# benjamincjackson/distance

Hardware: AMD Instinct MI355X
Metric: pairwise comparisons/sec (higher is better)
Workload: dtype u32

## Files before the change

distance_amd/_lib.py:

```python
from __future__ import annotations

import ctypes as C
import os
import re

_HERE = os.path.dirname(os.path.abspath(__file__))
LIB_PATH = os.environ.get("DST_LIB_PATH") or os.path.join(_HERE, "libdistance_hip.so")
HEADER_PATH = os.path.join(os.path.dirname(_HERE), "include", "distance_hip.h")

_u8p = C.POINTER(C.c_uint8)
_u32p = C.POINTER(C.c_uint32)
_u64p = C.POINTER(C.c_uint64)
_vp = C.c_void_p
ALLGATHER_FN = C.CFUNCTYPE(C.c_int, C.c_void_p, C.c_void_p, C.c_void_p, C.c_size_t, C.c_void_p)
SLAB_SINK = C.CFUNCTYPE(C.c_int, C.c_void_p, C.c_uint64, C.c_uint64, C.c_uint64, C.c_uint64, C.c_void_p)


class LaunchInfo(C.Structure):
    _fields_ = [("path", C.c_int), ("measure", C.c_int), ("family", C.c_int), ("out_kind", C.c_int), ("wide", C.c_int),
                ("square", C.c_int), ("event_waves", C.c_int), ("heavy_events", C.c_int), ("rows_per_tile", C.c_uint32),
                ("tile_cols", C.c_uint32), ("tiles", C.c_uint64), ("hot", C.c_int), ("run_records", C.c_int),
                ("variant", C.c_int), ("ksplit", C.c_uint32), ("pairs", C.c_uint64), ("events_per_pair", C.c_double),
                ("list_length", C.c_double), ("run_adds", C.c_double)]

# ... 54 lines not shown
    "dst_stream_open": (C.c_int, [_vp, C.c_int, C.c_int, C.c_size_t, C.c_int, C.POINTER(_vp)]),
    "dst_stream_open_wire": (C.c_int, [_vp, C.c_int, C.c_int, C.c_size_t, C.c_int, C.c_int, C.POINTER(_vp)]),
    "dst_stream_acquire": (C.c_int, [_vp, C.POINTER(_vp), C.POINTER(C.c_size_t), C.POINTER(_vp)]),
    "dst_stream_submit": (C.c_int, [_vp, C.c_size_t, C.c_int]),
    "dst_stream_collect": (C.c_int, [_vp, C.POINTER(C.c_size_t), C.POINTER(_vp)]),
    "dst_stream_in_flight": (C.c_int, [_vp]),
    "dst_stream_close": (C.c_int, [_vp]),
    "dst_comm_unique_id": (C.c_int, [_vp, C.c_size_t]),
    "dst_comm_create": (C.c_int, [_vp, _vp, C.c_int, C.c_int, C.POINTER(_vp)]),
    "dst_comm_create_custom": (C.c_int, [_vp, C.c_int, C.c_int, ALLGATHER_FN, _vp, C.POINTER(_vp)]),
    "dst_comm_destroy": (C.c_int, [_vp]),
    "dst_upload_shared": (C.c_int, [_vp, C.c_int, _vp, C.c_size_t, C.c_size_t, C.c_size_t, C.c_int, _vp]),
    "dst_shared_range": (C.c_int, [C.c_uint64, C.c_int, C.c_int, _u64p, _u64p]),
    "dst_shared_block_layout": (C.c_int, [C.c_uint64, C.c_int, C.c_uint32, _u32p]),
    "dst_shared_stats": (C.c_int, [_vp, C.c_int, _u64p, _u64p, _u64p]),
    "dst_comm_info": (C.c_int, [_vp, C.POINTER(C.c_int), C.POINTER(C.c_int)]),
    "dst_gather_slabs": (C.c_int, [_vp, _vp, _vp, _u64p, _u64p, C.c_int, _vp]),
    "dst_nearest": (C.c_int, [_vp, C.c_int, C.c_int, C.c_int, C.c_int, C.c_uint32, _vp, _vp, _vp, C.c_size_t, _u32p]),
    "dst_clusters": (C.c_int, [_vp, C.c_int, C.c_double, C.c_uint64, _vp, C.c_size_t, _u64p, _u64p]),
    "dst_nj": (C.c_int, [_vp, C.c_int, C.c_uint64, _vp, _vp, C.c_size_t]),
    "dst_nj_matrix": (C.c_int, [_vp, _vp, C.c_uint64, _vp, _vp, C.c_size_t]),
    "dst_newick": (C.c_int, [C.c_uint64, _vp, _vp, C.c_char_p, _vp, _vp, C.c_size_t, C.POINTER(C.c_size_t)]),
    "dst_newick_support": (C.c_int, [C.c_uint64, _vp, _vp, C.c_char_p, _vp, _vp, _vp, C.c_size_t,
                                     C.POINTER(C.c_size_t)]),
    "dst_bootstrap_columns": (None, [C.c_uint64, C.c_uint32, C.c_uint64, _vp]),
    "dst_nj_bootstrap": (C.c_int, [_vp, C.c_int, _vp, C.c_size_t, C.c_size_t, C.c_size_t, C.c_uint32, C.c_uint64,
                                   C.c_uint64, _vp, _vp, _vp, C.c_size_t]),
    "dst_host_alloc": (C.c_int, [C.c_size_t, C.POINTER(_vp)]),
    "dst_host_free": (C.c_int, [_vp]),
    "dst_out_bytes": (C.c_size_t, [C.c_int, C.c_int, C.c_uint64]),
# ... 35 lines not shown
```

distance_amd/csrc/dst_api.cpp:

```cpp
#include <algorithm>
#include <cmath>
#include <cstdio>
#include <cstdlib>
#include <cstring>
#include <memory>
#include <mutex>
#include <new>
#include <vector>

#include "dst_ctx.h"

using namespace dst;

namespace dst {

std::string g_create_err;
std::mutex g_create_mu;

int publish_prep(dst_ctx *ctx, hipStream_t stream);
int wait_for_other_runs(dst_ctx *ctx, hipStream_t stream);

int fail(dst_ctx *ctx, int status, const std::string &msg)
{
    if (ctx)
        ctx->err = msg;
    return status;
}

int fail_hip(dst_ctx *ctx, hipError_t e, const char *what)
{
    return fail(ctx, e == hipErrorOutOfMemory ? DST_ERR_NOMEM : DST_ERR_HIP,
                std::string(what) + ": " + hipGetErrorString(e));
}

// ... 88 lines not shown
            HIP_TRY(ctx, hipFree(b));
    s.ref.planes = nullptr;
    s.ref.hot_planes = nullptr;
    s.ref.hot_sites = nullptr;
    s.ref.stats = nullptr;
    s.ref.partials = nullptr;
    HIP_TRY(ctx, hipMalloc((void **)&s.ref.planes, 4 * s.nchunks * sizeof(uint4)));
    HIP_TRY(ctx, hipMalloc((void **)&s.ref.hot_planes, s.nchunks * sizeof(uint4)));
    HIP_TRY(ctx, hipMalloc((void **)&s.ref.hot_sites, s.nchunks * kChunkSites * sizeof(uint32_t)));
    HIP_TRY(ctx, hipMalloc((void **)&s.ref.stats, 8 * sizeof(uint64_t)));
    HIP_TRY(ctx, hipMalloc((void **)&s.ref.partials, s.nchunks * 16 * sizeof(uint32_t)));
    s.ref.nchunks = s.nchunks;
    return DST_OK;
}

bool planes_deferred_by_pack()
{
    static const bool keep = std::getenv("DST_PACK_ALL_PLANES") != nullptr;
    return !keep;
}

int pack_queue(dst_ctx *ctx, DeviceSet &s, const uint8_t *d_codes, size_t n, size_t len, size_t row_stride,
               const uint32_t *d_counts, unsigned long long *d_first_bad, hipStream_t stream, bool want_lists, bool nibbles)
{
    if (nibbles)
        want_lists = false;
    int rc = shape_set(ctx, s, n, len);
    if (rc)
        return rc;
    PackLists pl{};
    if (want_lists) {
        rc = alloc_ref(ctx, s);
        if (!rc && s.rec.pre_cap < n + 1) {
            if (s.rec.pre_cold)
                HIP_TRY(ctx, hipFree(s.rec.pre_cold));
            s.rec.pre_cold = s.rec.pre_hot = nullptr;
            s.rec.pre_totals = nullptr;
            s.rec.pre_cap = 0;
            const size_t words = 5 * (n + 1) + 8 + ((2 * (n + 1)) & 1);
            HIP_TRY(ctx, hipMalloc((void **)&s.rec.pre_cold, words * sizeof(uint32_t)));
            s.rec.pre_cap = n + 1;
        }
        if (!rc && s.runs.n_alloc < n + 1) {
            if (s.runs.index)
// ... 27 lines not shown
        pl.cnt_cold = s.rec.pre_cold;
        pl.cnt_hot = s.rec.pre_hot;
        pl.slots = s.rec.pre_slots;
        pl.defer_planes = planes_deferred_by_pack() ? 1 : 0;
        static const bool no_runs = std::getenv("DST_NO_RUN_RECORDS") != nullptr;
        if (!no_runs) {
            pl.cnt_run = s.runs.cnt_run;
            pl.run_cold = s.runs.run_cold;
            pl.run_hot = s.runs.run_hot;
        }
    }
    if (!want_lists)
        HIP_TRY(ctx, hipMemsetAsync(d_first_bad, 0xFF, sizeof(unsigned long long), stream));
    if (int rc_t = timer_begin(ctx, 1, stream))
        return rc_t;
    if (nibbles)
        HIP_TRY(ctx, launch_pack_nibbles(d_codes, row_stride, s, d_first_bad, stream));
    else
        HIP_TRY(ctx, launch_pack(d_codes, row_stride, s, d_first_bad, want_lists ? &pl : nullptr, stream));
    if (int rc_t = timer_end(ctx, 1, stream))
        return rc_t;
    if (d_counts) {
        HIP_TRY(ctx, hipMemsetAsync(s.counts, 0, s.npad * 4 * sizeof(uint32_t), stream));
        HIP_TRY(ctx, hipMemcpyAsync(s.counts, d_counts, n * 4 * sizeof(uint32_t),
                                    hipMemcpyDeviceToDevice, stream));
        s.have_counts = true;
    }
    return DST_OK;
}

int invalid_code_error(dst_ctx *ctx, unsigned long long first_bad, size_t len)
{
    char msg[160];
    std::snprintf(msg, sizeof msg,
// ... 6 lines not shown

int pack_set(dst_ctx *ctx, DeviceSet &s, const uint8_t *d_codes, size_t n, size_t len, size_t row_stride,
             const uint32_t *d_counts, hipStream_t stream);

int pack_from_device(dst_ctx *ctx, int slot, const uint8_t *d_codes, size_t n, size_t len,
                     size_t row_stride, const uint32_t *d_counts, hipStream_t stream)
{
    return pack_set(ctx, ctx->set[slot], d_codes, n, len, row_stride, d_counts, stream);
}

int pack_set(dst_ctx *ctx, DeviceSet &s, const uint8_t *d_codes, size_t n, size_t len, size_t row_stride,
             const uint32_t *d_counts, hipStream_t stream)
{
    const bool want_lists = ctx->path != DST_PATH_DENSE && n >= 2 && len > 0 && n < kEntryMask && len < kSiteMask &&
                            0.5 * (double)n * (double)n * (double)len >= ctx->prep_min_work;
    int rc = pack_queue(ctx, s, d_codes, n, len, row_stride, d_counts, ctx->d_first_bad, stream, want_lists);
    if (rc)
        return rc;
    const uint32_t max_run = (uint32_t)std::min<uint64_t>(n / 3, 24000000000ull / (32ull * std::max<size_t>(n, 1)));
    HIP_TRY(ctx, launch_report(ctx->d_first_bad,
                               want_lists ? reinterpret_cast<const unsigned long long *>(s.ref.stats) : nullptr,
                               want_lists ? s.rec.pre_cold : nullptr, want_lists ? s.rec.pre_hot : nullptr, n, ctx->d_report, stream,
                               want_lists ? &s.runs : nullptr, max_run, want_lists ? s.rec.pre_totals : nullptr));
    HIP_TRY(ctx, hipStreamSynchronize(stream));
    const unsigned long long first_bad = ctx->h_report[0], totals[2] = {ctx->h_report[9], ctx->h_report[10]};
    if (want_lists)
        for (int k = 0; k < 8; ++k)
            s.ref.h_stats[k] = ctx->h_report[1 + k];
    if (first_bad != ~0ull)
        return invalid_code_error(ctx, first_bad, len);
    s.loaded = true;
    if (want_lists) {
        s.ref.valid = true;
        const double max_dev = kListsMaxDeviation * (double)len * (double)std::min<size_t>(n, kRefSamples);
        s.rec.pre_valid = (double)s.ref.h_stats[1] <= (double)(unsigned long long)max_dev;
        s.lean = s.rec.pre_valid;
        s.planes_deferred = s.rec.pre_valid && planes_deferred_by_pack();
        s.rec.pre_epoch = s.epoch;
        s.rec.pre_total_cold = totals[0];
        s.rec.pre_total_hot = totals[1];
        s.runs.n_run = s.rec.pre_valid ? (uint32_t)ctx->h_report[11] : 0u;
        s.runs.removed = s.runs.n_run ? ctx->h_report[12] : 0;
        s.runs.active = s.runs.n_run != 0;
        s.runs.corr_family = -1;
    }
    return DST_OK;
}

int ensure_planes(dst_ctx *ctx, DeviceSet &s, hipStream_t stream)
{
    if (!s.planes_deferred)
        return DST_OK;
    if (s.partial)
        return fail(ctx, DST_ERR_STATE, "a set uploaded with dst_upload_shared runs on the consensus path only (its planes are "
                                        "not stored)");
    int rc = wait_for_other_runs(ctx, stream);
    if (rc)
        return rc;
    HIP_TRY(ctx, launch_planes_from_slots(s, stream));
// ... 873 lines not shown
                    ctx->text_num, (void *)ctx->text_len, (void *)ctx->text_scan, (void *)ctx->text_buf, (void *)ctx->text_flag, ctx->text_ties,
                    (void *)ctx->ids[0].off, (void *)ctx->ids[0].chars, (void *)ctx->ids[1].off, (void *)ctx->ids[1].chars, ctx->nn_slab, ctx->nn_lists,
                    ctx->cl_slab, ctx->cl_work})
        if (b)
            (void)hipFree(b);
    if (ctx->scratch)
        (void)hipFree(ctx->scratch);
    if (ctx->text_ties_host)
        (void)hipHostFree(ctx->text_ties_host);
    if (ctx->scratch_free)
        (void)hipEventDestroy(ctx->scratch_free);
    if (ctx->hot_free)
        (void)hipEventDestroy(ctx->hot_free);
    if (ctx->prep_event)
        (void)hipEventDestroy(ctx->prep_event);
    for (auto &r : ctx->recent)
        if (r.event)
            (void)hipEventDestroy(r.event);
    if (ctx->d_first_bad)
        (void)hipFree(ctx->d_first_bad);
    if (ctx->h_report)
        (void)hipHostFree(ctx->h_report);
    for (auto &t : ctx->timer)
        for (int k = 0; k < dst_ctx::kTimerRing; ++k) {
            if (t.begin[k])
                (void)hipEventDestroy(t.begin[k]);
            if (t.end[k])
                (void)hipEventDestroy(t.end[k]);
        }
    if (ctx->stream)
// ... 62 lines not shown
    plan_consensus_launch(measure, out_kind, wide != 0, square != 0, n_rows_in_launch, n_cols, total_pairs, events_per_pair,
                          list_length, run_adds, hot != 0, info);
    info->path = hot ? DST_PATH_HYBRID : DST_PATH_CONSENSUS;
    return DST_OK;
}

int dst_run_records(const dst_ctx *ctx, int slot, uint64_t *run_records, uint64_t *entries_removed)
{
    if (!ctx || slot < 0 || slot > 1)
        return DST_ERR_ARG;
    const DeviceSet &s = ctx->set[slot];
    if (run_records)
        *run_records = s.runs.active ? s.runs.n_run : 0;
    if (entries_removed)
        *entries_removed = s.runs.active ? s.runs.removed : 0;
    return DST_OK;
}

int dst_planes_stored(const dst_ctx *ctx, int slot, int *stored)
{
    if (!ctx || slot < 0 || slot > 1 || !stored)
        return DST_ERR_ARG;
    *stored = ctx->set[slot].loaded && !ctx->set[slot].planes_deferred ? 1 : 0;
    return DST_OK;
}

int dst_set_variant(dst_ctx *ctx, int variant)
{
    if (!ctx || variant < 0)
        return DST_ERR_ARG;
// ... 932 lines not shown
```

distance_amd/csrc/dst_consensus.hip:

```cpp
#include "dst_device.hpp"

#ifndef DST_OVF_DEPTH
#define DST_OVF_DEPTH 2
#endif

namespace dst {
namespace {

__device__ __forceinline__ int ref_class(uint32_t nib)
{
    return nib == 8 ? 0 : nib == 4 ? 1 : nib == 2 ? 2 : nib == 1 ? 3 : 4;
}

__device__ __forceinline__ uint32_t popc4(uint4 v)
{
    return __builtin_popcount(v.x) + __builtin_popcount(v.y) + __builtin_popcount(v.z) + __builtin_popcount(v.w);
}

__device__ __forceinline__ uint32_t sample_record(uint32_t k, uint32_t n, uint32_t samples)
{
    static_assert(kRefSamples == 512, "shifts below");
    return samples == n ? k : k * (n >> 9) + ((k * (n & 511u)) >> 9);
}

// ... 380 lines not shown
        sum += __shfl_xor(sum, 1);
        sum += __shfl_xor(sum, 2);
        sum += __shfl_xor(sum, 4);
        if (lane == 0 && sum)
            atomicAdd(total, (unsigned long long)sum);
    }
}

template <uint32_t CLN, bool WITHOUT_HOT>
__global__ __launch_bounds__(256) void slot_fill_kernel(const uint4 *__restrict__ slots, const uint4 *__restrict__ planes,
                                                        const uint4 *__restrict__ ref_planes,
                                                        const uint4 *__restrict__ hot_planes, uint32_t n,
                                                        uint32_t nchunks, uint32_t npad,
                                                        const uint32_t *__restrict__ rec_off, uint32_t *__restrict__ rec_ent,
                                                        uint32_t *__restrict__ range_start, uint32_t rec_first, uint32_t ent_cap,
                                                        const uint32_t *__restrict__ run_index, const uint32_t *__restrict__ run_state)
{
    constexpr uint32_t RLN = 64u / CLN;
    const uint32_t lane = threadIdx.x & 63u, wave = blockIdx.x * 4u + (threadIdx.x >> 6);
    const uint32_t rl = lane % RLN, cl = lane / RLN;
    const uint32_t r = rec_first + wave * RLN + rl;
    const bool live = r < n;
    const size_t ps = (size_t)nchunks * npad;
    uint32_t run = 0;
    const uint32_t base0 = live ? rec_off[r - rec_first] : 0u;
    const bool run_record = live && run_state && run_state[1] != 0 && run_index[r] != 0xFFFFFFFFu;
    const uint4 zero4 = make_uint4(0, 0, 0, 0);
    uint4 nslot = (live && cl < nchunks) ? slots[(size_t)cl * npad + r] : zero4;
    uint4 nslot2 = (live && cl + CLN < nchunks) ? slots[(size_t)(cl + CLN) * npad + r] : zero4;
    for (uint32_t c0 = 0; c0 < nchunks; c0 += CLN) {
        const uint32_t c = c0 + cl;
        const uint4 slot = nslot;
// ... 72 lines not shown
                }
            }
        }
        run += tot;
    }
}

constexpr uint32_t kBucketThreads = 1024;

constexpr uint32_t kBucketWalk = 8;
__global__ __launch_bounds__(kBucketThreads) void site_bucket_kernel(const uint32_t *__restrict__ rec_off,
                                                                     const uint32_t *__restrict__ rec_ent,
                                                                     const uint32_t *__restrict__ range_start, uint32_t n,
                                                                     uint32_t npad, uint32_t n_sites, uint4 *__restrict__ site_inl,
                                                                     uint32_t *__restrict__ site_ent,
                                                                     uint32_t *__restrict__ ovf_total)
{
    constexpr uint32_t NT = kBucketThreads, RPT = kPanelCols / NT;
    static_assert(NT == kBucketSites, "one bucket per thread in the offset scan");
    static_assert(RPT * NT == kPanelCols, "every record of the panel has its thread");
    __shared__ uint32_t cnt[kBucketSites];
    __shared__ uint32_t ooff[kBucketSites];
    __shared__ __attribute__((aligned(16))) uint16_t tabl[kBucketSites][16];
    __shared__ uint32_t wave_tot[NT / 64];
    __shared__ uint32_t blk_base;
    __shared__ uint32_t long_n, long_from[kPanelCols], long_to[kPanelCols];
    __shared__ uint16_t long_rec[kPanelCols];
    const uint32_t panel = blockIdx.y, tid = threadIdx.x, lane = tid & 63u;
    const uint32_t s0 = blockIdx.x * kBucketSites, ns = min(kBucketSites, n_sites - s0);
    const uint32_t r0 = panel * kPanelCols, nrec = min(kPanelCols, n - r0);
    cnt[tid] = 0;
    if (tid == 0)
// ... 321 lines not shown
        if ((threadIdx.x & 63u) == 0)
            part[threadIdx.x >> 6][k] = v[k];
    }
    __syncthreads();
    if (threadIdx.x < 4) {
        const unsigned long long t = part[0][threadIdx.x] + part[1][threadIdx.x] + part[2][threadIdx.x] + part[3][threadIdx.x];
        if (t)
            atomicAdd(&totals[threadIdx.x], t);
    }
}

__global__ __launch_bounds__(1024) void report_kernel(const unsigned long long *__restrict__ first_bad,
                                                      const unsigned long long *__restrict__ stats,
                                                      const unsigned long long *__restrict__ totals,
                                                      uint32_t *__restrict__ cnt0, uint32_t *__restrict__ cnt1, uint32_t n,
                                                      unsigned long long *report, RunsArg runs)
{
    __shared__ uint32_t wave_tot[16], base_s;
    __shared__ unsigned long long back[16][2];
    const uint32_t tid = threadIdx.x, lane = tid & 63u, wv = tid >> 6;
    unsigned long long cold = totals ? totals[0] : 0ull, hot = totals ? totals[1] : 0ull;
    const unsigned long long cand = totals && runs.cnt_run ? totals[2] : 0ull, cand_entries = totals ? totals[3] : 0ull;
    const bool strip = cand != 0 && cand <= runs.max_run;
    if (cand != 0) {
        if (tid == 0)
            base_s = 0;
        unsigned long long gave[2] = {0, 0};
        __syncthreads();
        for (uint32_t i0 = 0; i0 < n; i0 += 1024) {
            const uint32_t i = i0 + tid;
            const bool is_cand = i < n && runs.cnt_run[i] >= kRunMin;
            if (is_cand && !strip) {
                const uint32_t rc = runs.run_cold[i], rh = runs.run_hot[i];
                cnt0[i] += rc;
                cnt1[i] += rh;
                gave[0] += rc;
                gave[1] += rh;
// ... 40 lines not shown
        runs.state[0] = strip ? (uint32_t)cand : 0u;
        runs.state[1] = strip ? 1u : 0u;
    }
    if (tid == 0)
        report[0] = *first_bad;
    else if (tid <= 8)
        report[tid] = stats ? stats[tid - 1] : 0ull;
    else if (tid == 9)
        report[9] = cold;
    else if (tid == 10)
        report[10] = hot;
    else if (tid == 11)
        report[11] = strip ? cand : 0ull;
    else if (tid == 12)
        report[12] = strip ? cand_entries : 0ull;
}

struct RunConst {
    uint32_t *aent;
    size_t aent_stride;
    const uint32_t *index, *mask, *known;
    uint32_t mask_words;
};

__global__ __launch_bounds__(256) void aconst_kernel(const uint32_t *__restrict__ off,
                                                     const uint32_t *__restrict__ ent,
                                                     const ConsensusLut *__restrict__ lut, int family, int wide,
                                                     int words, uint32_t n, uint32_t npad,
                                                     uint32_t *__restrict__ aconst, RunConst rc)
{
// ... 1120 lines not shown
hipError_t launch_index(const DeviceSet &set, const uint4 *ref_planes, const uint4 *hot_planes, bool fill, bool skip_nclass,
                        uint32_t *rec, uint32_t *rec_ent, unsigned long long *total, hipStream_t stream, uint32_t *range_start)
{
    const unsigned blocks = (unsigned)((set.n + 31) / 32);
    if (fill)
        hipLaunchKernelGGL(index_kernel<true>, dim3(blocks), dim3(256), 0, stream, set.planes, ref_planes, hot_planes,
                           (uint32_t)set.n, (uint32_t)set.nchunks, (uint32_t)set.npad, skip_nclass ? 1 : 0, rec, rec_ent, total, range_start);
    else
        hipLaunchKernelGGL(index_kernel<false>, dim3(blocks), dim3(256), 0, stream, set.planes, ref_planes, hot_planes,
                           (uint32_t)set.n, (uint32_t)set.nchunks, (uint32_t)set.npad, skip_nclass ? 1 : 0, rec, rec_ent, total, range_start);
    return hipGetLastError();
}

hipError_t launch_slot_fill(const DeviceSet &set, const uint4 *ref_planes, const uint4 *hot_planes, bool without_hot,
                            uint32_t *rec_off, uint32_t *rec_ent, uint32_t *range_start, hipStream_t stream, size_t rec_begin,
                            size_t rec_end, uint32_t ent_cap)
{
    const uint32_t first = (uint32_t)std::min(rec_begin, set.n), n = (uint32_t)std::min(rec_end, set.n);
    const uint32_t nch = (uint32_t)set.nchunks, npad = (uint32_t)set.npad, count = n - first;
    if (n <= first)
        return hipSuccess;
    auto go = [&](auto cln, auto wh) {
        constexpr uint32_t CLN = decltype(cln)::value;
        constexpr uint32_t per_block = 4u * (64u / CLN);
        hipLaunchKernelGGL((slot_fill_kernel<CLN, decltype(wh)::value>), dim3((count + per_block - 1) / per_block), dim3(256), 0, stream,
                           set.rec.pre_slots, set.planes, ref_planes, hot_planes, n, nch, npad, rec_off, rec_ent, range_start, first,
                           ent_cap, set.runs.active ? set.runs.index : nullptr, set.runs.active ? set.runs.state : nullptr);
    };
    using std::integral_constant;
    const uint32_t cln = count >= 32768 ? 8u : count >= 16384 ? 16u : 32u;
    if (without_hot) {
        if (cln == 8) go(integral_constant<uint32_t, 8>{}, std::true_type{});
        else if (cln == 16) go(integral_constant<uint32_t, 16>{}, std::true_type{});
        else go(integral_constant<uint32_t, 32>{}, std::true_type{});
    } else {
        if (cln == 8) go(integral_constant<uint32_t, 8>{}, std::false_type{});
        else if (cln == 16) go(integral_constant<uint32_t, 16>{}, std::false_type{});
        else go(integral_constant<uint32_t, 32>{}, std::false_type{});
    }
    return hipGetLastError();
}

hipError_t launch_site_buckets(const DeviceSet &set, uint32_t n_panels, uint32_t *ovf_total, hipStream_t stream)
{
    const uint32_t n_sites = (uint32_t)(set.nchunks * kChunkSites);
    hipLaunchKernelGGL(site_bucket_kernel, dim3((n_sites + kBucketSites - 1) / kBucketSites, n_panels), dim3(kBucketThreads), 0,
                       stream, set.rec.off, set.rec.ent, set.rec.range_start, (uint32_t)set.n, (uint32_t)set.npad, n_sites, set.site.inl, set.site.ent,
                       ovf_total);
    return hipGetLastError();
}

size_t scan_tmp_words(size_t n)
{
    size_t words = 0;
    while (n > 1) {
        n = (n + kScanPerBlock - 1) / kScanPerBlock;
        words += n + 1;
    }
    return words + 2;
}

hipError_t launch_exclusive_scan(uint32_t *data, size_t n, uint32_t *tmp, hipStream_t stream, const uint32_t *src0,
                                 const uint32_t *src1, uint32_t *zero, uint32_t n_zero)
// ... 22 lines not shown
    e = launch_exclusive_scan(tmp, nb, tmp + nb + 1, stream);
    if (e != hipSuccess)
        return e;
    hipLaunchKernelGGL(scan_add_kernel, dim3((unsigned)nb), dim3(256), 0, stream, data, n, tmp);
    return hipGetLastError();
}

hipError_t launch_sum2_u32(const uint32_t *a0, const uint32_t *a1, size_t n, unsigned long long *totals, hipStream_t stream)
{
    hipLaunchKernelGGL(sum2_u32_kernel, dim3((unsigned)std::min<size_t>(256, (n + 1023) / 1024 + 1)), dim3(256), 0, stream, a0, a1, n, totals);
    return hipGetLastError();
}

hipError_t launch_report(const unsigned long long *first_bad, const unsigned long long *stats, uint32_t *cnt_cold,
                         uint32_t *cnt_hot, size_t n, unsigned long long *report, hipStream_t stream, const RunIndex *runs,
                         uint32_t max_run, unsigned long long *totals)
{
    RunsArg ra{nullptr, nullptr, nullptr, nullptr, nullptr, nullptr, 0};
    if (runs && runs->cnt_run)
        ra = RunsArg{runs->cnt_run, runs->run_cold, runs->run_hot, runs->index, runs->ids, runs->state, max_run};
    if (cnt_cold && totals) {
        const unsigned blocks = (unsigned)std::min<size_t>(128, (n + 255) / 256);
        hipLaunchKernelGGL(list_totals_kernel, dim3(blocks), dim3(256), 0, stream, cnt_cold, cnt_hot, (uint32_t)n, ra, totals);
    }
    hipLaunchKernelGGL(report_kernel, dim3(1), dim3(1024), 0, stream, first_bad, stats, cnt_cold && totals ? totals : nullptr, cnt_cold,
                       cnt_hot, (uint32_t)n, report, ra);
    return hipGetLastError();
}

hipError_t launch_aconst(const DeviceSet &set, int family, bool wide, const ConsensusLut *d_lut, hipStream_t stream)
{
    RunConst rc{nullptr, 0, nullptr, nullptr, nullptr, 0};
    if (set.runs.active)
        rc = RunConst{set.runs.aent, set.runs.aent_cap / (kMaxWords * sizeof(uint32_t)), set.runs.index, set.runs.mask, set.runs.known,
                      (uint32_t)set.runs.mask_words};
    hipLaunchKernelGGL(aconst_kernel, dim3((unsigned)((set.n + 3) / 4)), dim3(256), 0, stream, set.rec.off,
                       set.rec.ent, d_lut, family, wide ? 1 : 0, family_words(family, wide),
                       (uint32_t)set.n, (uint32_t)set.npad, set.aconst, rc);
    return hipGetLastError();
}

// ... 238 lines not shown
```

distance_amd/csrc/dst_ctx.h:

```cpp
#pragma once
#include <string>
#include <vector>

#include "dst_internal.h"

using namespace dst;

struct dst_ctx {
    int device = 0;
    hipStream_t stream = nullptr;
    DeviceSet set[2];
    DeviceSet boot;
    uint8_t *stage = nullptr;
    size_t stage_bytes = 0;
    unsigned long long *d_first_bad = nullptr;
    unsigned long long *h_report = nullptr, *d_report = nullptr;
    struct Schedule {
        bool square = false;
        uint64_t rb = 0, re = 0, ncols = 0;
        int bm = 0, bn = 0;
        uint32_t nblocks = 0;
        void *d_blocks = nullptr;
        size_t bytes = 0;
        uint64_t last_use = 0;
// ... 11 lines not shown
    uint32_t *scan_tmp = nullptr;
    size_t scan_tmp_bytes = 0;
    void *hot_tally = nullptr;
    size_t hot_tally_bytes = 0;
    hipEvent_t hot_free = nullptr;
    bool hot_used = false;
    hipEvent_t prep_event = nullptr;
    hipStream_t prep_stream = nullptr;
    bool prep_pending = false;
    struct Recent {
        hipStream_t stream = nullptr;
        hipEvent_t event = nullptr;
        bool used = false;
    } recent[4];
    unsigned recent_next = 0;
    void *host_out = nullptr;
    size_t host_out_bytes = 0;
    int ksplit = 0;
    uint32_t *scratch = nullptr;
    size_t scratch_bytes = 0;
    hipEvent_t scratch_free = nullptr;
    bool scratch_used = false;
    struct Ids {
        uint32_t *off = nullptr;
        char *chars = nullptr;
        size_t off_bytes = 0, chars_bytes = 0;
        uint64_t n = 0;
    } ids[2];
    void *text_res = nullptr;
    void *text_num = nullptr;
// ... 38 lines not shown
int fail(dst_ctx *ctx, int status, const std::string &msg);
int timer_begin(dst_ctx *ctx, int which, hipStream_t stream);
int timer_end(dst_ctx *ctx, int which, hipStream_t stream);
int fail_hip(dst_ctx *ctx, hipError_t e, const char *what);

#define HIP_TRY(ctx, call)                       \
    do {                                         \
        hipError_t e_ = (call);                  \
        if (e_ != hipSuccess)                    \
            return dst::fail_hip((ctx), e_, #call); \
    } while (0)

int ensure_bytes(dst_ctx *ctx, void **ptr, size_t *have, size_t want);
void free_set(DeviceSet &s);
int pack_queue(dst_ctx *ctx, DeviceSet &s, const uint8_t *d_codes, size_t n, size_t len, size_t row_stride,
               const uint32_t *d_counts, unsigned long long *d_first_bad, hipStream_t stream, bool want_lists, bool nibbles = false);
int invalid_code_error(dst_ctx *ctx, unsigned long long first_bad, size_t len);
int need_counts(dst_ctx *ctx, DeviceSet &s, hipStream_t stream);
int run_sets(dst_ctx *ctx, int measure, bool square, DeviceSet &rows, DeviceSet &cols, uint64_t rb, uint64_t re,
             int out_kind, void *d_out, size_t cap, void *stream_v);

}
```

distance_amd/csrc/dst_internal.h:

```cpp
#pragma once
#include <cstddef>
#include <cstdint>
#include <string>
#include <unordered_map>
#include <vector>

#include <hip/hip_runtime.h>

#include "../../include/distance_hip.h"

namespace dst {

enum Plane : int {
    PL_A = 0,
    PL_G = 1,
    PL_C = 2,
    PL_T = 3,
    PL_K = 4,
    PL_X1 = 5,
    PL_X0 = 6,
    PL_CL = 7,
    PL_COUNT = 8
};

// ... 170 lines not shown

hipError_t launch_shared_block(uint32_t *block, const SharedLayout &lay, const DeviceSet &set, size_t rec_begin, size_t count,
                               const uint32_t *off_local, const unsigned long long *first_bad, hipStream_t stream);
hipError_t launch_shared_splice(const uint32_t *gathered, const SharedLayout &lay, DeviceSet &set, uint32_t *len_all,
                                uint32_t *scan_tmp, bool with_counts, unsigned long long *report, hipStream_t stream);
hipError_t launch_ref_sample(const DeviceSet &set, hipStream_t stream);
hipError_t launch_ref_sample_bytes(const uint8_t *d_codes, size_t row_stride, const DeviceSet &set, hipStream_t stream,
                                   uint32_t *zero = nullptr, size_t zero_words = 0, unsigned long long *first_bad = nullptr);
hipError_t launch_hot_list(const DeviceSet &set, hipStream_t stream);
hipError_t launch_compact(const DeviceSet &src, const uint32_t *hot_sites, uint32_t n_hot, DeviceSet &dst, hipStream_t stream);
hipError_t launch_index(const DeviceSet &set, const uint4 *ref_planes, const uint4 *hot_planes, bool fill, bool skip_nclass,
                        uint32_t *rec_off_or_cnt, uint32_t *rec_ent, unsigned long long *total,
                        hipStream_t stream, uint32_t *range_start = nullptr);
hipError_t launch_slot_fill(const DeviceSet &set, const uint4 *ref_planes, const uint4 *hot_planes, bool without_hot,
                            uint32_t *rec_off, uint32_t *rec_ent, uint32_t *range_start, hipStream_t stream, size_t rec_begin = 0,
                            size_t rec_end = ~(size_t)0, uint32_t ent_cap = 0xFFFFFFFFu);
hipError_t launch_site_buckets(const DeviceSet &set, uint32_t n_panels, uint32_t *ovf_total, hipStream_t stream);
size_t scan_tmp_words(size_t n);
hipError_t launch_exclusive_scan(uint32_t *data, size_t n, uint32_t *tmp, hipStream_t stream, const uint32_t *src0 = nullptr,
                                 const uint32_t *src1 = nullptr, uint32_t *zero = nullptr, uint32_t n_zero = 0);
hipError_t launch_aconst(const DeviceSet &set, int family, bool wide, const ConsensusLut *d_lut, hipStream_t stream);
hipError_t launch_run_known(const DeviceSet &set, const uint4 *ref_planes, const uint4 *hot_planes, hipStream_t stream);
hipError_t launch_run_masks(const DeviceSet &set, hipStream_t stream);
hipError_t launch_run_tables(const DeviceSet &set, int family, bool wide, bool without_hot, const ConsensusLut *d_lut, hipStream_t stream);
constexpr int kReportWords = 13;
hipError_t launch_report(const unsigned long long *first_bad, const unsigned long long *stats, uint32_t *cnt_cold,
                         uint32_t *cnt_hot, size_t n, unsigned long long *report, hipStream_t stream, const RunIndex *runs = nullptr,
                         uint32_t max_run = 0, unsigned long long *totals = nullptr);
hipError_t launch_sum2_u32(const uint32_t *a0, const uint32_t *a1, size_t n, unsigned long long *totals, hipStream_t stream);
hipError_t launch_consensus_pairs(int measure, const ConsensusLaunch &cl, const uint32_t f_words[kMaxWords],
                                  hipStream_t stream);
int consensus_event_waves(int measure, int out_kind, bool wide, int heavy_events);
hipError_t launch_site_hist(const DeviceSet &set, uint32_t *hist, hipStream_t stream);

const char *consensus_build_flags();

struct PackLists {
    const uint4 *ref_planes, *hot_planes;
    const unsigned long long *stats;
    unsigned long long max_dev_sum;
    uint32_t *cnt_cold, *cnt_hot;
    uint4 *slots;
    uint32_t *cnt_run, *run_cold, *run_hot;
// ... 86 lines not shown
```

distance_amd/csrc/dst_shared.cpp:

```cpp
#include <algorithm>
#include <cstdio>

#include "dst_ctx.h"

using namespace dst;

namespace dst {
dst_ctx *comm_ctx(dst_comm *c);
int comm_rank(const dst_comm *c);
int comm_world(const dst_comm *c);
int comm_allgather(dst_comm *c, const void *d_send, void *d_recv, size_t bytes, hipStream_t stream);
int pack_from_device(dst_ctx *ctx, int slot, const uint8_t *d_codes, size_t n, size_t len, size_t row_stride,
                     const uint32_t *d_counts, hipStream_t stream);
int shape_set(dst_ctx *ctx, DeviceSet &s, size_t n, size_t len);
int alloc_ref(dst_ctx *ctx, DeviceSet &s);
int ensure_lut(dst_ctx *ctx);
int wait_for_other_runs(dst_ctx *ctx, hipStream_t stream);
int publish_prep(dst_ctx *ctx, hipStream_t stream);
}

extern "C" int dst_upload_shared(dst_comm *comm, int slot, const void *d_codes_v, size_t n, size_t len, size_t row_stride,
                                 int with_counts, void *stream_v)
{
    if (!comm)
        return DST_ERR_ARG;
    dst_ctx *ctx = comm_ctx(comm);
    const int rank = comm_rank(comm), world = comm_world(comm);
    const uint8_t *d_codes = static_cast<const uint8_t *>(d_codes_v);
    if (slot < 0 || slot > 1)
        return fail(ctx, DST_ERR_ARG, "slot must be 0 or 1");
    if (n == 0)
        return fail(ctx, DST_ERR_ARG, "Empty FASTA file");
    if ((len && !d_codes) || row_stride < len)
        return fail(ctx, DST_ERR_ARG, "null codes or row_stride < len");
    if (n >= 0xFFFFFE00ull || len >= 0xFFFFFF00ull)
        return fail(ctx, DST_ERR_ARG, "n and len must fit 32 bits");
    HIP_TRY(ctx, hipSetDevice(ctx->device));
    hipStream_t stream = stream_v ? (hipStream_t)stream_v : ctx->stream;
    const bool eligible = (ctx->path == DST_PATH_AUTO || ctx->path == DST_PATH_CONSENSUS) && n >= 2 && len > 0 &&
                          n < kEntryMask && len < kSiteMask;
    if (!eligible)
        return pack_from_device(ctx, slot, d_codes, n, len, row_stride, nullptr, stream);
    DeviceSet &s = ctx->set[slot];
    dst_ctx::Shared &sh = ctx->shared[slot];
    int rc = wait_for_other_runs(ctx, stream);
    if (!rc)
        rc = ensure_lut(ctx);
    if (!rc)
        rc = shape_set(ctx, s, n, len);
    if (!rc)
        rc = alloc_ref(ctx, s);
    if (rc)
        return rc;
    SharedLayout lay = shared_layout(n, world, 0);
    const uint64_t want_cap = sh.last_biggest ? sh.last_biggest + sh.last_biggest / 4 + 4096 : (uint64_t)lay.rmax * 96 + 16384;
    if (want_cap * (uint64_t)world >= 0x7FFFFFF0ull)
        return pack_from_device(ctx, slot, d_codes, n, len, row_stride, nullptr, stream);
    lay = shared_layout(n, world, (uint32_t)want_cap);
    const size_t rec_begin = std::min<size_t>(n, (size_t)rank * lay.rmax), rec_end = std::min<size_t>(n, ((size_t)rank + 1) * lay.rmax);
    const size_t count = rec_end - rec_begin;
// ... 116 lines not shown
```

distance_amd/engine.py:

```python
from __future__ import annotations

import ctypes as C

import numpy as np

from ._lib import ALLGATHER_FN, SLAB_SINK, DistanceError, LaunchInfo, load

MEASURES = {"n": 0, "n_high": 1, "raw": 2, "jc69": 3, "k80": 4, "tn93": 5}
INT_MEASURES = ("n", "n_high")
FLOAT_MEASURES = ("raw", "jc69", "k80", "tn93")
OUT_DISTANCE, OUT_TALLY, OUT_TALLY16 = 0, 1, 2
FIN_CLOSE = 0x100
PATHS = {"auto": 0, "dense": 1, "consensus": 2, "hybrid": 3}
MATRIX_STYLES = {"tsv": 0, "phylip": 1}


def _measure_id(measure) -> int:
    if isinstance(measure, str):
        m = load().dst_measure_from_name(measure.encode())
        if m < 0:
            raise ValueError(f"Unknown distance measure {measure!r}")
        return m
    return int(measure)

# ... 237 lines not shown

    def upload_device(self, slot: int, d_ptr: int, n: int, length: int, row_stride: int,
                      d_counts_ptr: int | None = None, stream: int | None = None):
        self._check(self._lib.dst_upload_device(self._h, slot, d_ptr, n, length, row_stride, d_counts_ptr,
                                                stream))

    def upload_shared(self, comm: "Comm", slot: int, d_ptr: int, n: int, length: int, row_stride: int,
                      with_counts: bool = False, stream: int | None = None):
        self._check(self._lib.dst_upload_shared(comm._h, slot, d_ptr, n, length, row_stride, int(with_counts), stream))

    def shared_stats(self, slot: int = 0) -> dict:
        a, b, c = C.c_uint64(), C.c_uint64(), C.c_uint64()
        self._check(self._lib.dst_shared_stats(self._h, slot, C.byref(a), C.byref(b), C.byref(c)))
        return {"shared_uploads": int(a.value), "fallbacks": int(b.value), "block_entries": int(c.value)}

    def set_info(self, slot: int) -> tuple[int, int]:
        n, length = C.c_size_t(), C.c_size_t()
        self._check(self._lib.dst_set_info(self._h, slot, C.byref(n), C.byref(length)))
        return int(n.value), int(length.value)

    def base_counts(self, slot: int) -> np.ndarray:
        n, _ = self.set_info(slot)
        out = np.zeros((n, 4), np.uint32)
        self._check(self._lib.dst_get_base_counts(self._h, slot, out.ctypes.data))
        return out

    def _alloc(self, m: int, out_kind: int, pairs: int) -> np.ndarray:
        if out_kind == OUT_TALLY:
            return np.zeros((pairs, self._lib.dst_tally_width(m)), np.uint32)
        if out_kind == OUT_TALLY16:
# ... 304 lines not shown
```

include/distance_hip.h:

```cpp
#ifndef DISTANCE_HIP_H
#define DISTANCE_HIP_H

#include <stddef.h>
#include <stdint.h>

#ifdef __cplusplus
extern "C" {
#endif

#define DST_ABI_VERSION 3

typedef struct dst_ctx dst_ctx;

typedef enum {
    DST_N = 0,
    DST_N_HIGH = 1,
    DST_RAW = 2,
    DST_JC69 = 3,
    DST_K80 = 4,
    DST_TN93 = 5
} dst_measure;

typedef enum {
    DST_OK = 0,
// ... 15 lines not shown
const char *dst_status_string(int status);
const char *dst_build_flags(void);

int dst_create(int device, dst_ctx **ctx);
int dst_destroy(dst_ctx *ctx);
const char *dst_last_error(const dst_ctx *ctx);
int dst_set_variant(dst_ctx *ctx, int variant);
int dst_variant_count(int measure);
int dst_set_ksplit(dst_ctx *ctx, int ksplit);

int dst_set_prep_threshold(dst_ctx *ctx, double site_comparisons);
typedef enum { DST_PATH_AUTO = 0, DST_PATH_DENSE = 1, DST_PATH_CONSENSUS = 2, DST_PATH_HYBRID = 3 } dst_path;
int dst_set_path(dst_ctx *ctx, int path);
int dst_run_records(const dst_ctx *ctx, int slot, uint64_t *run_records, uint64_t *entries_removed);
int dst_planes_stored(const dst_ctx *ctx, int slot, int *stored);
int dst_last_path(const dst_ctx *ctx);
typedef struct {
    int path;
    int measure;
    int family;
    int out_kind;
    int wide;
    int square;
    int event_waves;
    int heavy_events;
    uint32_t rows_per_tile;
    uint32_t tile_cols;
    uint64_t tiles;
    int hot;
    int run_records;
// ... 119 lines not shown
```

Baseline: 448.0 billion.

## Queue sparse-list prep on the upload stream behind a device-side skip flag

```diff
diff --git a/distance_amd/_lib.py b/distance_amd/_lib.py
--- a/distance_amd/_lib.py
+++ b/distance_amd/_lib.py
@@ -92,6 +92,7 @@
     "dst_shared_range": (C.c_int, [C.c_uint64, C.c_int, C.c_int, _u64p, _u64p]),
     "dst_shared_block_layout": (C.c_int, [C.c_uint64, C.c_int, C.c_uint32, _u32p]),
     "dst_shared_stats": (C.c_int, [_vp, C.c_int, _u64p, _u64p, _u64p]),
+    "dst_prep_stats": (C.c_int, [_vp, _u64p, _u64p, _u32p]),
     "dst_comm_info": (C.c_int, [_vp, C.POINTER(C.c_int), C.POINTER(C.c_int)]),
     "dst_gather_slabs": (C.c_int, [_vp, _vp, _vp, _u64p, _u64p, C.c_int, _vp]),
     "dst_nearest": (C.c_int, [_vp, C.c_int, C.c_int, C.c_int, C.c_int, C.c_uint32, _vp, _vp, _vp, C.c_size_t, _u32p]),
diff --git a/distance_amd/csrc/dst_api.cpp b/distance_amd/csrc/dst_api.cpp
--- a/distance_amd/csrc/dst_api.cpp
+++ b/distance_amd/csrc/dst_api.cpp
@@ -18,6 +18,7 @@
 std::mutex g_create_mu;
 
 int publish_prep(dst_ctx *ctx, hipStream_t stream);
+int order_after_prep(dst_ctx *ctx, hipStream_t stream);
 int wait_for_other_runs(dst_ctx *ctx, hipStream_t stream);
 
 int fail(dst_ctx *ctx, int status, const std::string &msg)
@@ -136,6 +137,45 @@
     return DST_OK;
 }
 
+constexpr uint64_t kPrepFirstGuess = 96;
+
+bool prep_queued_with_upload()
+{
+    return std::getenv("DST_SERIAL_PREP") == nullptr;
+}
+
+int ensure_lut(dst_ctx *ctx);
+
+int prep_queue_alloc(dst_ctx *ctx, DeviceSet &s, uint64_t *ent_cap)
+{
+    dst_ctx::PrepQueue &pp = ctx->pipe;
+    if (!pp.reported) {
+        HIP_TRY(ctx, hipEventCreateWithFlags(&pp.reported, hipEventDisableTiming));
+        HIP_TRY(ctx, hipMalloc((void **)&pp.skip, sizeof(uint32_t)));
+    }
+    int rc = ensure_lut(ctx);
+    if (rc)
+        return rc;
+    const uint32_t n_panels = (uint32_t)((s.n + kPanelCols - 1) / kPanelCols);
+    const size_t n_buckets = s.nchunks * kChunkSites * (size_t)n_panels;
+    const uint64_t guess = std::max<uint64_t>(kPrepFirstGuess * s.n, pp.ent_high + pp.ent_high / 8);
+    const size_t want = (size_t)std::min<uint64_t>(guess, 0x7FFFFFFFull / 4);
+    rc = ensure_bytes(ctx, (void **)&s.rec.off, &s.rec.off_cap, (s.n + 1) * sizeof(uint32_t));
+    if (!rc)
+        rc = ensure_bytes(ctx, (void **)&ctx->scan_tmp, &ctx->scan_tmp_bytes, scan_tmp_words(s.n + 1) * sizeof(uint32_t));
+    if (!rc)
+        rc = ensure_bytes(ctx, (void **)&s.site.inl, &s.site.inl_cap, std::max<size_t>(n_buckets, 1) * 2 * sizeof(uint4));
+    if (!rc)
+        rc = ensure_bytes(ctx, (void **)&s.rec.ent, &s.rec.ent_cap, (want + 4) * sizeof(uint32_t));
+    if (!rc)
+        rc = ensure_bytes(ctx, (void **)&s.site.ent, &s.site.ent_cap, want * sizeof(uint32_t));
+    if (!rc)
+        rc = ensure_bytes(ctx, (void **)&s.rec.range_start, &s.rec.range_cap,
+                          ((s.nchunks * kChunkSites + kBucketSites - 1) / kBucketSites) * s.npad * sizeof(uint32_t));
+    *ent_cap = std::min<uint64_t>(std::min<uint64_t>(s.rec.ent_cap / sizeof(uint32_t) - 4, s.site.ent_cap / sizeof(uint32_t)), 0x7FFFFFFFull / 4);
+    return rc;
+}
+
 bool planes_deferred_by_pack()
 {
     static const bool keep = std::getenv("DST_PACK_ALL_PLANES") != nullptr;
@@ -143,13 +183,29 @@
 }
 
 int pack_queue(dst_ctx *ctx, DeviceSet &s, const uint8_t *d_codes, size_t n, size_t len, size_t row_stride,
-               const uint32_t *d_counts, unsigned long long *d_first_bad, hipStream_t stream, bool want_lists, bool nibbles)
+               const uint32_t *d_counts, unsigned long long *d_first_bad, hipStream_t stream, bool want_lists, bool nibbles,
+               bool queue_lists, uint64_t *ent_cap)
 {
     if (nibbles)
         want_lists = false;
-    int rc = shape_set(ctx, s, n, len);
+    int rc = order_after_prep(ctx, stream);
+    if (!rc)
+        rc = shape_set(ctx, s, n, len);
     if (rc)
         return rc;
+    {
+        const size_t n_buckets = s.nchunks * kChunkSites * ((n + kPanelCols - 1) / kPanelCols);
+        if (!want_lists || !ent_cap || n_buckets >= 0xFFFFFFFFull || n_buckets * 2 * sizeof(uint4) > (16ull << 30))
+            queue_lists = false;
+    }
+    ctx->pipe.last_queued = queue_lists ? 1u : 0u;
+    if (queue_lists) {
+        rc = prep_queue_alloc(ctx, s, ent_cap);
+        if (!rc)
+            rc = wait_for_other_runs(ctx, stream);
+        if (rc)
+            return rc;
+    }
     PackLists pl{};
     if (want_lists) {
         rc = alloc_ref(ctx, s);
@@ -207,10 +263,11 @@
         HIP_TRY(ctx, hipMemsetAsync(d_first_bad, 0xFF, sizeof(unsigned long long), stream));
     if (int rc_t = timer_begin(ctx, 1, stream))
         return rc_t;
-    if (nibbles)
+    if (nibbles) {
         HIP_TRY(ctx, launch_pack_nibbles(d_codes, row_stride, s, d_first_bad, stream));
-    else
+    } else {
         HIP_TRY(ctx, launch_pack(d_codes, row_stride, s, d_first_bad, want_lists ? &pl : nullptr, stream));
+    }
     if (int rc_t = timer_end(ctx, 1, stream))
         return rc_t;
     if (d_counts) {
@@ -247,15 +304,32 @@
 {
     const bool want_lists = ctx->path != DST_PATH_DENSE && n >= 2 && len > 0 && n < kEntryMask && len < kSiteMask &&
                             0.5 * (double)n * (double)n * (double)len >= ctx->prep_min_work;
-    int rc = pack_queue(ctx, s, d_codes, n, len, row_stride, d_counts, ctx->d_first_bad, stream, want_lists);
+    uint64_t ent_cap = 0;
+    int rc = pack_queue(ctx, s, d_codes, n, len, row_stride, d_counts, ctx->d_first_bad, stream, want_lists, false,
+                        want_lists && prep_queued_with_upload(), &ent_cap);
     if (rc)
         return rc;
+    const bool queued = ctx->pipe.last_queued != 0;
+    const unsigned long long max_dev_sum = (unsigned long long)(kListsMaxDeviation * (double)len * (double)std::min<size_t>(n, kRefSamples));
     const uint32_t max_run = (uint32_t)std::min<uint64_t>(n / 3, 24000000000ull / (32ull * std::max<size_t>(n, 1)));
     HIP_TRY(ctx, launch_report(ctx->d_first_bad,
                                want_lists ? reinterpret_cast<const unsigned long long *>(s.ref.stats) : nullptr,
                                want_lists ? s.rec.pre_cold : nullptr, want_lists ? s.rec.pre_hot : nullptr, n, ctx->d_report, stream,
-                               want_lists ? &s.runs : nullptr, max_run, want_lists ? s.rec.pre_totals : nullptr));
-    HIP_TRY(ctx, hipStreamSynchronize(stream));
+                               want_lists ? &s.runs : nullptr, max_run, want_lists ? s.rec.pre_totals : nullptr, queued ? ent_cap : ~0ull,
+                               max_dev_sum, queued ? ctx->pipe.skip : nullptr));
+    if (queued) {
+        HIP_TRY(ctx, hipEventRecord(ctx->pipe.reported, stream));
+        uint32_t *const counters = reinterpret_cast<uint32_t *>(ctx->d_total);
+        HIP_TRY(ctx, launch_exclusive_scan(s.rec.off, s.n + 1, ctx->scan_tmp, stream, s.rec.pre_cold, s.rec.pre_hot, counters, 4));
+        HIP_TRY(ctx, launch_slot_fill(s, s.ref.planes, s.ref.hot_planes, false, s.rec.off, s.rec.ent, s.rec.range_start, stream, 0,
+                                      ~(size_t)0, (uint32_t)ent_cap, ctx->pipe.skip));
+        HIP_TRY(ctx, launch_site_buckets(s, (uint32_t)((n + kPanelCols - 1) / kPanelCols), counters + 2, stream, ctx->pipe.skip));
+        if (int rc_p = publish_prep(ctx, stream))
+            return rc_p;
+        HIP_TRY(ctx, hipEventSynchronize(ctx->pipe.reported));
+    } else {
+        HIP_TRY(ctx, hipStreamSynchronize(stream));
+    }
     const unsigned long long first_bad = ctx->h_report[0], totals[2] = {ctx->h_report[9], ctx->h_report[10]};
     if (want_lists)
         for (int k = 0; k < 8; ++k)
@@ -276,6 +350,22 @@
         s.runs.removed = s.runs.n_run ? ctx->h_report[12] : 0;
         s.runs.active = s.runs.n_run != 0;
         s.runs.corr_family = -1;
+        if (s.rec.pre_valid)
+            ctx->pipe.ent_high = std::max<uint64_t>(ctx->pipe.ent_high, totals[0] + totals[1]);
+        if (queued && s.rec.pre_valid) {
+            if (ctx->h_report[13] == 0) {
+                s.rec.total = totals[0] + totals[1];
+                s.rec.valid = s.rec.ranges_valid = s.site.valid = true;
+                s.rec.ref_owner = &s;
+                s.rec.ref_epoch = s.epoch;
+                s.rec.without_hot = false;
+                s.site.n_panels = (uint32_t)((n + kPanelCols - 1) / kPanelCols);
+                s.aconst_family = -1;
+                ctx->pipe.uploads += 1;
+            } else {
+                ctx->pipe.fallbacks += 1;
+            }
+        }
     }
     return DST_OK;
 }
@@ -1179,6 +1269,10 @@
         (void)hipEventDestroy(ctx->hot_free);
     if (ctx->prep_event)
         (void)hipEventDestroy(ctx->prep_event);
+    if (ctx->pipe.reported)
+        (void)hipEventDestroy(ctx->pipe.reported);
+    if (ctx->pipe.skip)
+        (void)hipFree(ctx->pipe.skip);
     for (auto &r : ctx->recent)
         if (r.event)
             (void)hipEventDestroy(r.event);
@@ -1271,6 +1365,19 @@
         *run_records = s.runs.active ? s.runs.n_run : 0;
     if (entries_removed)
         *entries_removed = s.runs.active ? s.runs.removed : 0;
+    return DST_OK;
+}
+
+int dst_prep_stats(const dst_ctx *ctx, uint64_t *queued_uploads, uint64_t *fallbacks, uint32_t *last_queued)
+{
+    if (!ctx)
+        return DST_ERR_ARG;
+    if (queued_uploads)
+        *queued_uploads = ctx->pipe.uploads;
+    if (fallbacks)
+        *fallbacks = ctx->pipe.fallbacks;
+    if (last_queued)
+        *last_queued = ctx->pipe.last_queued;
     return DST_OK;
 }
 
diff --git a/distance_amd/csrc/dst_consensus.hip b/distance_amd/csrc/dst_consensus.hip
--- a/distance_amd/csrc/dst_consensus.hip
+++ b/distance_amd/csrc/dst_consensus.hip
@@ -418,8 +418,11 @@
                                                         uint32_t nchunks, uint32_t npad,
                                                         const uint32_t *__restrict__ rec_off, uint32_t *__restrict__ rec_ent,
                                                         uint32_t *__restrict__ range_start, uint32_t rec_first, uint32_t ent_cap,
-                                                        const uint32_t *__restrict__ run_index, const uint32_t *__restrict__ run_state)
-{
+                                                        const uint32_t *__restrict__ run_index, const uint32_t *__restrict__ run_state,
+                                                        const uint32_t *__restrict__ skip)
+{
+    if (skip && *skip)
+        return;
     constexpr uint32_t RLN = 64u / CLN;
     const uint32_t lane = threadIdx.x & 63u, wave = blockIdx.x * 4u + (threadIdx.x >> 6);
     const uint32_t rl = lane % RLN, cl = lane / RLN;
@@ -522,8 +525,11 @@
                                                                      const uint32_t *__restrict__ range_start, uint32_t n,
                                                                      uint32_t npad, uint32_t n_sites, uint4 *__restrict__ site_inl,
                                                                      uint32_t *__restrict__ site_ent,
-                                                                     uint32_t *__restrict__ ovf_total)
-{
+                                                                     uint32_t *__restrict__ ovf_total,
+                                                                     const uint32_t *__restrict__ skip)
+{
+    if (skip && *skip)
+        return;
     constexpr uint32_t NT = kBucketThreads, RPT = kPanelCols / NT;
     static_assert(NT == kBucketSites, "one bucket per thread in the offset scan");
     static_assert(RPT * NT == kPanelCols, "every record of the panel has its thread");
@@ -875,13 +881,17 @@
                                                       const unsigned long long *__restrict__ stats,
                                                       const unsigned long long *__restrict__ totals,
                                                       uint32_t *__restrict__ cnt0, uint32_t *__restrict__ cnt1, uint32_t n,
-                                                      unsigned long long *report, RunsArg runs)
+                                                      unsigned long long *report, RunsArg runs, unsigned long long ent_cap,
+                                                      unsigned long long max_dev_sum, uint32_t *__restrict__ lists_skip)
 {
     __shared__ uint32_t wave_tot[16], base_s;
     __shared__ unsigned long long back[16][2];
     const uint32_t tid = threadIdx.x, lane = tid & 63u, wv = tid >> 6;
     unsigned long long cold = totals ? totals[0] : 0ull, hot = totals ? totals[1] : 0ull;
     const unsigned long long cand = totals && runs.cnt_run ? totals[2] : 0ull, cand_entries = totals ? totals[3] : 0ull;
+    const bool lists_stand = totals && stats && cold + hot <= ent_cap && cand == 0 && stats[1] <= max_dev_sum;
+    if (lists_skip && tid == 0)
+        *lists_skip = lists_stand ? 0u : 1u;
     const bool strip = cand != 0 && cand <= runs.max_run;
     if (cand != 0) {
         if (tid == 0)
@@ -952,6 +962,8 @@
         report[11] = strip ? cand : 0ull;
     else if (tid == 12)
         report[12] = strip ? cand_entries : 0ull;
+    else if (tid == 13)
+        report[13] = lists_stand ? 0ull : 1ull;
 }
 
 struct RunConst {
@@ -2102,7 +2114,7 @@
 
 hipError_t launch_slot_fill(const DeviceSet &set, const uint4 *ref_planes, const uint4 *hot_planes, bool without_hot,
                             uint32_t *rec_off, uint32_t *rec_ent, uint32_t *range_start, hipStream_t stream, size_t rec_begin,
-                            size_t rec_end, uint32_t ent_cap)
+                            size_t rec_end, uint32_t ent_cap, const uint32_t *skip)
 {
     const uint32_t first = (uint32_t)std::min(rec_begin, set.n), n = (uint32_t)std::min(rec_end, set.n);
     const uint32_t nch = (uint32_t)set.nchunks, npad = (uint32_t)set.npad, count = n - first;
@@ -2113,7 +2125,7 @@
         constexpr uint32_t per_block = 4u * (64u / CLN);
         hipLaunchKernelGGL((slot_fill_kernel<CLN, decltype(wh)::value>), dim3((count + per_block - 1) / per_block), dim3(256), 0, stream,
                            set.rec.pre_slots, set.planes, ref_planes, hot_planes, n, nch, npad, rec_off, rec_ent, range_start, first,
-                           ent_cap, set.runs.active ? set.runs.index : nullptr, set.runs.active ? set.runs.state : nullptr);
+                           ent_cap, set.runs.active ? set.runs.index : nullptr, set.runs.active ? set.runs.state : nullptr, skip);
     };
     using std::integral_constant;
     const uint32_t cln = count >= 32768 ? 8u : count >= 16384 ? 16u : 32u;
@@ -2129,12 +2141,12 @@
     return hipGetLastError();
 }
 
-hipError_t launch_site_buckets(const DeviceSet &set, uint32_t n_panels, uint32_t *ovf_total, hipStream_t stream)
+hipError_t launch_site_buckets(const DeviceSet &set, uint32_t n_panels, uint32_t *ovf_total, hipStream_t stream, const uint32_t *skip)
 {
     const uint32_t n_sites = (uint32_t)(set.nchunks * kChunkSites);
     hipLaunchKernelGGL(site_bucket_kernel, dim3((n_sites + kBucketSites - 1) / kBucketSites, n_panels), dim3(kBucketThreads), 0,
                        stream, set.rec.off, set.rec.ent, set.rec.range_start, (uint32_t)set.n, (uint32_t)set.npad, n_sites, set.site.inl, set.site.ent,
-                       ovf_total);
+                       ovf_total, skip);
     return hipGetLastError();
 }
 
@@ -2187,7 +2199,8 @@
 
 hipError_t launch_report(const unsigned long long *first_bad, const unsigned long long *stats, uint32_t *cnt_cold,
                          uint32_t *cnt_hot, size_t n, unsigned long long *report, hipStream_t stream, const RunIndex *runs,
-                         uint32_t max_run, unsigned long long *totals)
+                         uint32_t max_run, unsigned long long *totals, unsigned long long ent_cap, unsigned long long max_dev_sum,
+                         uint32_t *lists_skip)
 {
     RunsArg ra{nullptr, nullptr, nullptr, nullptr, nullptr, nullptr, 0};
     if (runs && runs->cnt_run)
@@ -2197,7 +2210,7 @@
         hipLaunchKernelGGL(list_totals_kernel, dim3(blocks), dim3(256), 0, stream, cnt_cold, cnt_hot, (uint32_t)n, ra, totals);
     }
     hipLaunchKernelGGL(report_kernel, dim3(1), dim3(1024), 0, stream, first_bad, stats, cnt_cold && totals ? totals : nullptr, cnt_cold,
-                       cnt_hot, (uint32_t)n, report, ra);
+                       cnt_hot, (uint32_t)n, report, ra, ent_cap, max_dev_sum, lists_skip);
     return hipGetLastError();
 }
 
diff --git a/distance_amd/csrc/dst_ctx.h b/distance_amd/csrc/dst_ctx.h
--- a/distance_amd/csrc/dst_ctx.h
+++ b/distance_amd/csrc/dst_ctx.h
@@ -49,6 +49,13 @@
         bool used = false;
     } recent[4];
     unsigned recent_next = 0;
+    struct PrepQueue {
+        hipEvent_t reported = nullptr;
+        uint32_t *skip = nullptr;
+        uint64_t ent_high = 0;
+        uint64_t uploads = 0, fallbacks = 0;
+        uint32_t last_queued = 0;
+    } pipe;
     void *host_out = nullptr;
     size_t host_out_bytes = 0;
     int ksplit = 0;
@@ -117,7 +124,8 @@
 int ensure_bytes(dst_ctx *ctx, void **ptr, size_t *have, size_t want);
 void free_set(DeviceSet &s);
 int pack_queue(dst_ctx *ctx, DeviceSet &s, const uint8_t *d_codes, size_t n, size_t len, size_t row_stride,
-               const uint32_t *d_counts, unsigned long long *d_first_bad, hipStream_t stream, bool want_lists, bool nibbles = false);
+               const uint32_t *d_counts, unsigned long long *d_first_bad, hipStream_t stream, bool want_lists, bool nibbles = false,
+               bool queue_lists = false, uint64_t *ent_cap = nullptr);
 int invalid_code_error(dst_ctx *ctx, unsigned long long first_bad, size_t len);
 int need_counts(dst_ctx *ctx, DeviceSet &s, hipStream_t stream);
 int run_sets(dst_ctx *ctx, int measure, bool square, DeviceSet &rows, DeviceSet &cols, uint64_t rb, uint64_t re,
diff --git a/distance_amd/csrc/dst_internal.h b/distance_amd/csrc/dst_internal.h
--- a/distance_amd/csrc/dst_internal.h
+++ b/distance_amd/csrc/dst_internal.h
@@ -208,8 +208,9 @@
                         hipStream_t stream, uint32_t *range_start = nullptr);
 hipError_t launch_slot_fill(const DeviceSet &set, const uint4 *ref_planes, const uint4 *hot_planes, bool without_hot,
                             uint32_t *rec_off, uint32_t *rec_ent, uint32_t *range_start, hipStream_t stream, size_t rec_begin = 0,
-                            size_t rec_end = ~(size_t)0, uint32_t ent_cap = 0xFFFFFFFFu);
-hipError_t launch_site_buckets(const DeviceSet &set, uint32_t n_panels, uint32_t *ovf_total, hipStream_t stream);
+                            size_t rec_end = ~(size_t)0, uint32_t ent_cap = 0xFFFFFFFFu, const uint32_t *skip = nullptr);
+hipError_t launch_site_buckets(const DeviceSet &set, uint32_t n_panels, uint32_t *ovf_total, hipStream_t stream,
+                               const uint32_t *skip = nullptr);
 size_t scan_tmp_words(size_t n);
 hipError_t launch_exclusive_scan(uint32_t *data, size_t n, uint32_t *tmp, hipStream_t stream, const uint32_t *src0 = nullptr,
                                  const uint32_t *src1 = nullptr, uint32_t *zero = nullptr, uint32_t n_zero = 0);
@@ -217,10 +218,11 @@
 hipError_t launch_run_known(const DeviceSet &set, const uint4 *ref_planes, const uint4 *hot_planes, hipStream_t stream);
 hipError_t launch_run_masks(const DeviceSet &set, hipStream_t stream);
 hipError_t launch_run_tables(const DeviceSet &set, int family, bool wide, bool without_hot, const ConsensusLut *d_lut, hipStream_t stream);
-constexpr int kReportWords = 13;
+constexpr int kReportWords = 14;
 hipError_t launch_report(const unsigned long long *first_bad, const unsigned long long *stats, uint32_t *cnt_cold,
                          uint32_t *cnt_hot, size_t n, unsigned long long *report, hipStream_t stream, const RunIndex *runs = nullptr,
-                         uint32_t max_run = 0, unsigned long long *totals = nullptr);
+                         uint32_t max_run = 0, unsigned long long *totals = nullptr, unsigned long long ent_cap = ~0ull,
+                         unsigned long long max_dev_sum = ~0ull, uint32_t *lists_skip = nullptr);
 hipError_t launch_sum2_u32(const uint32_t *a0, const uint32_t *a1, size_t n, unsigned long long *totals, hipStream_t stream);
 hipError_t launch_consensus_pairs(int measure, const ConsensusLaunch &cl, const uint32_t f_words[kMaxWords],
                                   hipStream_t stream);
diff --git a/distance_amd/csrc/dst_shared.cpp b/distance_amd/csrc/dst_shared.cpp
--- a/distance_amd/csrc/dst_shared.cpp
+++ b/distance_amd/csrc/dst_shared.cpp
@@ -17,6 +17,7 @@
 int ensure_lut(dst_ctx *ctx);
 int wait_for_other_runs(dst_ctx *ctx, hipStream_t stream);
 int publish_prep(dst_ctx *ctx, hipStream_t stream);
+int order_after_prep(dst_ctx *ctx, hipStream_t stream);
 }
 
 extern "C" int dst_upload_shared(dst_comm *comm, int slot, const void *d_codes_v, size_t n, size_t len, size_t row_stride,
@@ -44,6 +45,8 @@
     DeviceSet &s = ctx->set[slot];
     dst_ctx::Shared &sh = ctx->shared[slot];
     int rc = wait_for_other_runs(ctx, stream);
+    if (!rc)
+        rc = order_after_prep(ctx, stream);
     if (!rc)
         rc = ensure_lut(ctx);
     if (!rc)
diff --git a/distance_amd/engine.py b/distance_amd/engine.py
--- a/distance_amd/engine.py
+++ b/distance_amd/engine.py
@@ -275,6 +275,11 @@
         self._check(self._lib.dst_shared_stats(self._h, slot, C.byref(a), C.byref(b), C.byref(c)))
         return {"shared_uploads": int(a.value), "fallbacks": int(b.value), "block_entries": int(c.value)}
 
+    def prep_stats(self) -> dict:
+        a, b, c = C.c_uint64(), C.c_uint64(), C.c_uint32()
+        self._check(self._lib.dst_prep_stats(self._h, C.byref(a), C.byref(b), C.byref(c)))
+        return {"queued_uploads": int(a.value), "fallbacks": int(b.value), "last_queued": int(c.value)}
+
     def set_info(self, slot: int) -> tuple[int, int]:
         n, length = C.c_size_t(), C.c_size_t()
         self._check(self._lib.dst_set_info(self._h, slot, C.byref(n), C.byref(length)))
diff --git a/include/distance_hip.h b/include/distance_hip.h
--- a/include/distance_hip.h
+++ b/include/distance_hip.h
@@ -53,6 +53,7 @@
 int dst_set_path(dst_ctx *ctx, int path);
 int dst_run_records(const dst_ctx *ctx, int slot, uint64_t *run_records, uint64_t *entries_removed);
 int dst_planes_stored(const dst_ctx *ctx, int slot, int *stored);
+int dst_prep_stats(const dst_ctx *ctx, uint64_t *queued_uploads, uint64_t *fallbacks, uint32_t *last_queued);
 int dst_last_path(const dst_ctx *ctx);
 typedef struct {
     int path;
```

Result: no change. 450.3 billion, median of 6 (+0.5%).
